# juwangvsu/cartographer-1

Measured on AMD Instinct MI355X. Metric: loop-closure constraint candidates/sec (node x submap pairs) + ms/scan-match, 2D 5cm grid, higher is better.
Workload: dtype u8

## Files before the change

cartographer-1_amd/csrc/csm_device.h:

```cpp
#ifndef CSM_DEVICE_H_
#define CSM_DEVICE_H_

#include <cstdint>

#if defined(__HIPCC__)
#define CSM_HD __host__ __device__
#else
#define CSM_HD
#endif

namespace csm {

constexpr int kMaxLevels = 12;
constexpr int kNumXcd = 8;
constexpr int kSearchThreads = 256;
constexpr int kWaves = kSearchThreads / 64;
constexpr int kStackCap = 160;
constexpr int kTopChunk = 64;
constexpr int kMaxPoints = 16448;
constexpr int kIndexLimit = 16383;
constexpr int kOffsetLimit = 8191;
constexpr int kMaxRotations = 16383;
constexpr int16_t kSentinel = -32768;

struct SubmapDesc {
  double max_x, max_y, resolution;
  int32_t nx, ny;
  int32_t levels;
  int32_t pad0;
  const uint8_t* level[kMaxLevels];
  int32_t wide_nx[kMaxLevels];
  int32_t wide_ny[kMaxLevels];
  int32_t zero_index[kMaxLevels];
  const uint32_t* quad[kMaxLevels];
  const uint8_t* pyramid_base;
  int32_t pyramid_bytes;
  int32_t quad_off[kMaxLevels];
  int32_t quad_pws[kMaxLevels];
  int32_t quad_pph[kMaxLevels];
  int32_t quad_w[kMaxLevels];
  int32_t quad_h[kMaxLevels];
  int32_t quad_bytes[kMaxLevels];
  int32_t cshift[kMaxLevels];
  int32_t quad_bias[kMaxLevels];
  int32_t quad_es[kMaxLevels];
  int32_t hex_mask;
};

constexpr int kMaxClusterShift = 3;

constexpr int kHexEntryBytes = 16;

struct PairDesc {
  int32_t submap;
  int32_t num_points;
  int64_t point_offset;
  int32_t rot_offset;
  int32_t num_scans;
  int32_t num_linear;
  int32_t max_rejected_sum;
  float tx, ty;
  float pre_w, pre_s;
  int32_t collect;
  int32_t collect_sum;
};

struct ScoreJob {
  int32_t pair, rot, first, count;
};
constexpr int kTieCap = 4096;

struct WalkJob2 {
  int32_t pair;
  int32_t target_sum;
  int32_t top_level;
  int32_t top_first;
  int32_t top_count;
  int32_t bounds_first;
  float min_s, max_s;
};
constexpr int kWalkStack = 64;

struct WorkQueues {
  const int32_t* pair_order;
  const int64_t* chunk_prefix;
  int32_t queue_begin[kNumXcd + 1];
  int64_t queue_chunks[kNumXcd];
  int32_t rot_chunk;
};

struct WorkQueues2 {
  const int32_t* pair_order;
  const int64_t* chunk_prefix;
  const int32_t* block_first;
  int32_t block_offset[kNumXcd];
  int32_t queue_begin[kNumXcd + 1];
  int64_t queue_chunks[kNumXcd];
  int32_t rot_chunk;
};

#ifndef CSM_MAX_ROT_CHUNK
#define CSM_MAX_ROT_CHUNK 16
#endif
constexpr int kV4MaxRotChunk = CSM_MAX_ROT_CHUNK;

constexpr int kStack2 = 1024;
constexpr int kSpill2 = 7168;
constexpr int kBatchNodes = 64;

constexpr int kSumShift = 42;
constexpr uint64_t kTieMask = (uint64_t(1) << kSumShift) - 1;

CSM_HD inline uint64_t PackLeafKey(uint32_t sum, int rot, int xo, int yo) {
  const uint64_t idx = (uint64_t(rot) << 28) | (uint64_t(xo + 8192) << 14) |
                       uint64_t(yo + 8192);
  return (uint64_t(sum) << kSumShift) | (~idx & kTieMask);
}
CSM_HD inline uint64_t HighLeafKey(uint64_t key) {
  return (key & ~kTieMask) | (~key & kTieMask);
}
CSM_HD inline void UnpackLeafKey(uint64_t key, uint32_t* sum, int* rot, int* xo, int* yo) {
  *sum = static_cast<uint32_t>(key >> kSumShift);
  const uint64_t idx = ~key & kTieMask;
  *rot = static_cast<int>(idx >> 28);
  *xo = static_cast<int>((idx >> 14) & 0x3fff) - 8192;
  *yo = static_cast<int>(idx & 0x3fff) - 8192;
}

constexpr int kStatHighWater = 2 + 2 * kMaxLevels + 4;
constexpr int kStatLines = kStatHighWater + 1;
constexpr int kStatsWords = kStatLines + 5 * kMaxLevels;

constexpr int32_t kStatusRange = 1;

}

#endif
```

cartographer-1_amd/csrc/csm_host.cc:

```cpp

#include <hip/hip_runtime.h>

#include <algorithm>
#include <atomic>
#include <chrono>
#include <cmath>
#include <cstdlib>
#include <cstring>
#include <limits>
#include <map>
#include <memory>
#include <mutex>
#include <set>
#include <thread>
#include <array>
#include <tuple>
#include <vector>

#include "../../include/csm_amd.h"
#include "csm_device.h"
#include "csm_internal.h"
#include "csm_launch.h"
#include "parallel_sort.h"
#include "search_window.h"

namespace csm {



namespace {


int AutoSearchDepth(int configured, int nx, int ny) {
  int d = configured;
  const int span = std::max(nx, ny);
  while (d < kMaxLevels && (1 << (d - 1)) < span / 2) ++d;
  return std::max(d, configured);
}

void ClusterShifts(int32_t* out) {
  static const int kDefault[kMaxLevels] = {0, 0, 2, 2, 2, 3, 3, 3, 3, 3, 3, 3};
  for (int l = 0; l < kMaxLevels; ++l) out[l] = kDefault[l];
  if (const char* env = std::getenv("CSM_CLUSTER")) {
    int l = 0;
    for (const char* c = env; *c && l < kMaxLevels; ++l) {
      out[l] = std::atoi(c);
      while (*c && *c != ',') ++c;
      if (*c == ',') ++c;
    }
    for (; l < kMaxLevels; ++l) out[l] = out[l - 1];
  }
  for (int l = 0; l < kMaxLevels; ++l)
    out[l] = std::max(0, std::min({out[l], l, kMaxClusterShift}));
}

}
}

using namespace csm;


namespace {

int EnsureDevice(csm_context* ctx) {
  return hipSetDevice(ctx->device) == hipSuccess ? CSM_OK : CSM_EHIP;
}

}

namespace csm {

namespace {
std::mutex& PoolRegistryMutex() {
  static std::mutex m;
  return m;
}
std::vector<BufPool*>& PoolRegistry() {
  static std::vector<BufPool*> r;
  return r;
}
}

BufPool::BufPool() {
  std::lock_guard<std::mutex> g(PoolRegistryMutex());
  PoolRegistry().push_back(this);
}

BufPool::~BufPool() {
  {
    std::lock_guard<std::mutex> g(PoolRegistryMutex());
    auto& r = PoolRegistry();
    r.erase(std::remove(r.begin(), r.end(), this), r.end());
  }
  Release();
}

void BufPool::Release() {
  std::lock_guard<std::mutex> g(mu_);
  for (auto& b : bufs_) (void)hipFree(b.first);
  bufs_.clear();
  held_ = 0;
}

int BufPool::Take(size_t n, DevBuf* out) {
  {
    std::lock_guard<std::mutex> g(mu_);
    int best = -1;
    for (int i = 0; i < static_cast<int>(bufs_.size()); ++i) {
      const size_t b = bufs_[i].second;
      if (b >= n && b <= 2 * n + 4096 && (best < 0 || b < bufs_[best].second)) best = i;
    }
    if (best >= 0) {
      out->ptr = bufs_[best].first;
      out->bytes = bufs_[best].second;
      held_ -= bufs_[best].second;
      bufs_.erase(bufs_.begin() + best);
      return CSM_OK;
    }
  }
  return out->Reserve(n);
}

void BufPool::Give(DevBuf* b) {
  constexpr size_t kMaxPooled = 8192;
  if (!b->ptr) return;
  std::lock_guard<std::mutex> g(mu_);
  bufs_.emplace_back(b->ptr, b->bytes);
  held_ += b->bytes;
  b->ptr = nullptr;
  b->bytes = 0;
  size_t drop = 0;
  while (drop < bufs_.size() && (bufs_.size() - drop > kMaxPooled || held_ > cap_bytes_)) {
    held_ -= bufs_[drop].second;
    (void)hipFree(bufs_[drop].first);
    ++drop;
  }
  bufs_.erase(bufs_.begin(), bufs_.begin() + static_cast<std::ptrdiff_t>(drop));
}

void ReleaseIdlePools() {
  std::lock_guard<std::mutex> g(PoolRegistryMutex());
  for (BufPool* p : PoolRegistry()) p->Release();
}

csm_context* AcquireCallContext(csm_context* owner) {
  {
    std::lock_guard<std::mutex> g(owner->call_mu);
    if (!owner->call_free.empty()) {
      csm_context* c = owner->call_free.back();
      owner->call_free.pop_back();
      c->timing = owner->timing.load();
      return c;
    }
  }
  csm_context* c = nullptr;
  if (csm_context_create(owner->device, &c) != CSM_OK) return nullptr;
  c->call_owner = owner;
  c->timing = owner->timing.load();
  std::lock_guard<std::mutex> g(owner->call_mu);
  owner->call_all.push_back(c);
  return c;
}

void ReleaseCallContext(csm_context* owner, csm_context* c) {
  if (!c) return;
  std::lock_guard<std::mutex> g(owner->call_mu);
  AddTiming(&owner->call_t, c->t);
  c->t = csm_timing{};
  owner->call_free.push_back(c);
}

}

namespace {

const std::pair<SearchWindow2D, std::vector<ZRot>>& WindowFor(
    csm_scan_set* s, int scan, double lin, double ang, double res) {
  const auto key = std::make_tuple(scan, ang, lin, res);
  auto it = s->windows.find(key);
  if (it != s->windows.end()) return it->second;
  const int64_t b = s->offsets[scan], e = s->offsets[scan + 1];
  SearchWindow2D w = MakeSearchWindow2D(lin, ang, s->host_points.data() + 3 * b,
                                        static_cast<int32_t>(e - b), res, nullptr);
  std::vector<ZRot> table;
  RotationTable(w, &table);
  return s->windows.emplace(key, std::make_pair(w, std::move(table))).first->second;
}

struct SearchPlan {
  bool use_v2 = true, hex = false, fifo = true;
  int rc = 2, max_npad = 64;
};

int LaunchSearch(csm_context* ctx, csm_scan_set* scans, const std::vector<PairDesc>& pdesc,
                 const std::vector<uint64_t>* init_best, const SearchPlan& plan, bool timed,
                 std::vector<uint64_t>* keys, std::vector<uint64_t>* keys_hi,
                 std::vector<int32_t>* stat, unsigned long long* stats_host,
                 std::vector<uint2>* ties = nullptr, std::vector<int32_t>* tie_counts = nullptr) {
  const int np = static_cast<int>(pdesc.size());
  const int rc = plan.rc;
  static const bool spread_on = [] {
    const char* e = std::getenv("CSM_QUEUE_SPREAD");
    return !(e && std::atoi(e) == 0);
  }();
  int nsub = 0;
  for (int i = 0; i < np; ++i) nsub = std::max(nsub, pdesc[i].submap + 1);
  const int reps = spread_on && nsub > 0 && nsub < kNumXcd ? kNumXcd / nsub : 1;
  std::vector<int32_t> seen(reps > 1 ? nsub : 0, 0);
  std::vector<std::vector<int32_t>> q(kNumXcd);
  for (int i = 0; i < np; ++i) {
    const int sm = pdesc[i].submap;
    const int qi = reps > 1 ? sm + nsub * (seen[sm]++ % reps) : sm % kNumXcd;
    q[qi].push_back(i);
  }
  std::vector<int32_t> order;
  std::vector<int64_t> prefix;
  WorkQueues wq{};
  wq.rot_chunk = rc;
  int64_t running = 0;
  for (int x = 0; x < kNumXcd; ++x) {
    std::stable_sort(q[x].begin(), q[x].end(),
                     [&](int a, int b) { return pdesc[a].submap < pdesc[b].submap; });
    wq.queue_begin[x] = static_cast<int32_t>(order.size());
    const int64_t qstart = running;
    for (int pi : q[x]) {
      order.push_back(pi);
      prefix.push_back(running);
      running += (pdesc[pi].num_scans + rc - 1) / rc;
    }
    wq.queue_chunks[x] = running - qstart;
  }
  wq.queue_begin[kNumXcd] = static_cast<int32_t>(order.size());
  prefix.push_back(running);

  std::vector<int32_t> blocks;
  WorkQueues2 wq2{};
  if (plan.use_v2) {
    wq2.rot_chunk = rc;
    for (int x = 0; x < kNumXcd; ++x) {
      wq2.queue_begin[x] = wq.queue_begin[x];
      wq2.queue_chunks[x] = wq.queue_chunks[x];
      wq2.block_offset[x] = static_cast<int32_t>(blocks.size());
      const int64_t qstart = prefix[wq.queue_begin[x]];
      int e = wq.queue_begin[x];
      for (int64_t c = 0; c < wq.queue_chunks[x]; c += 64) {
        while (prefix[e + 1] - qstart <= c) ++e;
        blocks.push_back(e);
      }
    }
    wq2.queue_begin[kNumXcd] = wq.queue_begin[kNumXcd];
  }

  auto align = [](size_t v) { return (v + 255) & ~size_t{255}; };
  size_t at = 0;
  auto region = [&](size_t bytes) {
    const size_t o = at;
    at = align(at + std::max<size_t>(bytes, 1));
    return o;
  };
  const size_t o_pd = region(sizeof(PairDesc) * np), o_order = region(sizeof(int32_t) * order.size()),
               o_prefix = region(sizeof(int64_t) * prefix.size()),
               o_blocks = region(sizeof(int32_t) * blocks.size());
  const size_t o_best = region(sizeof(uint64_t) * np), o_hi = region(sizeof(uint64_t) * np),
               o_status = region(sizeof(int32_t) * np), o_tcount = region(sizeof(int32_t) * np),
               o_counters = region(sizeof(unsigned long long) * kNumXcd);
  const size_t o_stats = region(sizeof(unsigned long long) * kStatsWords);
  const size_t arena_bytes = at;
  const size_t in_end = init_best ? o_hi : o_best;
  const size_t zero_begin = in_end;
  int rcode;
  if ((rcode = ctx->arena.Reserve(arena_bytes))) return rcode;
  if ((rcode = ctx->arena_in.Reserve(in_end))) return rcode;
  if ((rcode = ctx->arena_out.Reserve(arena_bytes - o_best))) return rcode;
  if (ties && (rcode = ctx->ties.Reserve(sizeof(uint2) * kTieCap * static_cast<size_t>(np))))
    return rcode;
  char* hin = ctx->arena_in.as<char>();
  std::memcpy(hin + o_pd, pdesc.data(), sizeof(PairDesc) * np);
  std::memcpy(hin + o_order, order.data(), sizeof(int32_t) * order.size());
  std::memcpy(hin + o_prefix, prefix.data(), sizeof(int64_t) * prefix.size());
  if (!blocks.empty()) std::memcpy(hin + o_blocks, blocks.data(), sizeof(int32_t) * blocks.size());
  if (init_best) std::memcpy(hin + o_best, init_best->data(), sizeof(uint64_t) * np);
  char* dev = ctx->arena.as<char>();
  hipStream_t st = ctx->stream;
  CSM_HIP(hipMemcpyAsync(dev, hin, in_end, hipMemcpyHostToDevice, st));
  CSM_HIP(hipMemsetAsync(dev + zero_begin, 0, arena_bytes - zero_begin, st));
  ctx->pair_desc_dev = dev + o_pd;
  PairDesc* d_pairs = reinterpret_cast<PairDesc*>(dev + o_pd);
  uint64_t* d_best = reinterpret_cast<uint64_t*>(dev + o_best);
  uint64_t* d_hi = reinterpret_cast<uint64_t*>(dev + o_hi);
  int32_t* d_status = reinterpret_cast<int32_t*>(dev + o_status);
  int32_t* d_tcount = reinterpret_cast<int32_t*>(dev + o_tcount);
  unsigned long long* d_counters = reinterpret_cast<unsigned long long*>(dev + o_counters);
  unsigned long long* d_stats = reinterpret_cast<unsigned long long*>(dev + o_stats);
  wq.pair_order = reinterpret_cast<int32_t*>(dev + o_order);
  wq.chunk_prefix = reinterpret_cast<int64_t*>(dev + o_prefix);

  const int64_t total_chunks = running;
  const int max_npad = plan.max_npad;
  if (timed) CSM_HIP(hipEventRecord(ctx->ev0, st));
  if (plan.use_v2) {
    wq2.pair_order = wq.pair_order;
    wq2.chunk_prefix = wq.chunk_prefix;
    wq2.block_first = reinterpret_cast<int32_t*>(dev + o_blocks);
    int capc = (3 * max_npad / 4 + 63) & ~63;
    if (const char* ce = std::getenv("CSM_CAPC_PCT"))
      capc = std::max(64, (std::atoi(ce) * max_npad / 100 + 63) & ~63);
    const int lds_cap = 96 * 1024;
    auto dyn_bytes = [&](int cap) { return static_cast<size_t>(rc) * (max_npad * 4 + cap * 5); };
    while (capc > 0 && dyn_bytes(capc) > lds_cap) capc -= 64;
    const size_t dyn_lds = (dyn_bytes(capc) + 15) & ~size_t{15};
    int per_cu = std::max(1, std::min(8, Fast2dSearchV2BlocksPerCu(plan.hex, plan.fifo, dyn_lds)));
    if (const char* w = std::getenv("CSM_WG_PER_CU")) per_cu = std::max(1, std::min(per_cu, std::atoi(w)));
    if (std::getenv("CSM_PROFILE2D") && !init_best)
      std::fprintf(stderr, "fast2d launch: %s %s, %d rotations per item, %zu B dynamic LDS (capc %d), %d workgroups per CU\n",
                   plan.hex ? "v5" : "v4", plan.fifo ? "fifo" : "lifo", rc, dyn_lds, capc, per_cu);
    const int64_t full = static_cast<int64_t>(ctx->num_cus) * per_cu;
    const int64_t share = std::max<int64_t>(ctx->num_cus, full / std::max(1, ctx->grid_share));
    const int grid = static_cast<int>(std::min<int64_t>(share, std::max<int64_t>(total_chunks, 1)));
    if ((rcode = ctx->spill.Reserve(sizeof(uint2) * kSpill2 * static_cast<size_t>(grid))))
      return rcode;
    CSM_HIP(LaunchFast2dSearchV2(grid, dyn_lds, st, ctx->submap_desc.as<SubmapDesc>(), d_pairs,
                                 scans->points.as<float>(), scans->rot_dev.as<float2>(), wq2,
                                 d_counters, d_best, d_status, d_stats, ctx->spill.as<uint2>(),
                                 max_npad, capc, plan.hex, plan.fifo, d_hi,
                                 ties ? ctx->ties.as<uint2>() : nullptr, d_tcount, ties != nullptr));
  } else {
    const size_t dyn_lds = static_cast<size_t>(rc) * max_npad * sizeof(uint32_t);
    const int grid = static_cast<int>(std::min<int64_t>(static_cast<int64_t>(ctx->num_cus) * 4,
                                                        std::max<int64_t>(total_chunks, 1)));
    CSM_HIP(LaunchFast2dSearch(grid, dyn_lds, st, ctx->submap_desc.as<SubmapDesc>(), d_pairs,
                               scans->points.as<float>(), scans->rot_dev.as<float2>(), wq,
                               d_counters, d_best, d_status, d_stats));
  }
  if (timed) CSM_HIP(hipEventRecord(ctx->ev1, st));
  char* hout = ctx->arena_out.as<char>();
  CSM_HIP(hipMemcpyAsync(hout, dev + o_best, arena_bytes - o_best, hipMemcpyDeviceToHost, st));
  if (ties) {
    ties->resize(static_cast<size_t>(kTieCap) * np);
    CSM_HIP(hipMemcpyAsync(ties->data(), ctx->ties.ptr, sizeof(uint2) * ties->size(),
                           hipMemcpyDeviceToHost, st));
  }
  CSM_HIP(hipStreamSynchronize(st));
  auto out = [&](size_t o) { return hout + (o - o_best); };
  keys->assign(reinterpret_cast<uint64_t*>(out(o_best)), reinterpret_cast<uint64_t*>(out(o_best)) + np);
  keys_hi->assign(reinterpret_cast<uint64_t*>(out(o_hi)), reinterpret_cast<uint64_t*>(out(o_hi)) + np);
  stat->assign(reinterpret_cast<int32_t*>(out(o_status)), reinterpret_cast<int32_t*>(out(o_status)) + np);
  std::memcpy(stats_host, out(o_stats), sizeof(unsigned long long) * kStatsWords);
  if (ties)
    tie_counts->assign(reinterpret_cast<int32_t*>(out(o_tcount)),
                       reinterpret_cast<int32_t*>(out(o_tcount)) + np);
  return CSM_OK;
}

void RotationBounds(const csm_scan_set* scans, const PairDesc& d, const SubmapDesc& sm,
                    const ZRot& rot, int b[4]) {
  int mnx = 0x7fffffff, mxx = -0x7fffffff, mny = 0x7fffffff, mxy = -0x7fffffff;
  const ZRot pre{d.pre_w, d.pre_s};
  const float* p = scans->host_points.data() + 3 * d.point_offset;
  for (int i = 0; i < d.num_points; ++i) {
    float x, y;
    RotateZ(pre, p[3 * i], p[3 * i + 1], &x, &y);
    RotateZ(rot, x, y, &x, &y);
    const float px = d.tx + x, py = d.ty + y;
    const int ix = static_cast<int>(std::round((sm.max_y - static_cast<double>(py)) / sm.resolution - 0.5));
    const int iy = static_cast<int>(std::round((sm.max_x - static_cast<double>(px)) / sm.resolution - 0.5));
    mnx = std::min(mnx, ix); mxx = std::max(mxx, ix);
    mny = std::min(mny, iy); mxy = std::max(mxy, iy);
  }
  b[0] = std::max(-d.num_linear, std::min(0, -mxx));
  b[1] = std::min(d.num_linear, std::max(0, sm.nx - 1 - mnx));
  b[2] = std::max(-d.num_linear, std::min(0, -mxy));
  b[3] = std::min(d.num_linear, std::max(0, sm.ny - 1 - mny));
}

int ResolveTies(csm_context* ctx, csm_fast2d* const* submaps, csm_scan_set* scans,
                const std::vector<PairDesc>& pdesc, const std::vector<float2>& rot_host,
                const SearchPlan& plan, std::vector<int32_t>* stat,
                const std::vector<uint64_t>& keys_hi, std::vector<uint64_t>* keys,
                std::vector<int8_t>* tie_code) {
  std::vector<int> tied;
  for (int k = 0; k < static_cast<int>(pdesc.size()); ++k) {
    const uint64_t key = (*keys)[k];
    if (((*stat)[k] & kStatusRange) || key == 0) continue;
    const int64_t sum = static_cast<int64_t>(key >> kSumShift);
    if (sum <= pdesc[k].max_rejected_sum) continue;
    if ((keys_hi[k] >> kSumShift) == (key >> kSumShift) && keys_hi[k] != HighLeafKey(key))
      tied.push_back(k);
  }
  if (tied.empty()) return CSM_OK;
  ctx->t.tied_pairs += static_cast<int64_t>(tied.size());
  const bool prof = std::getenv("CSM_PROFILE2D") != nullptr;
  auto now = [] { return std::chrono::steady_clock::now(); };
  auto ms = [](std::chrono::steady_clock::time_point a, std::chrono::steady_clock::time_point b) {
    return std::chrono::duration<double, std::milli>(b - a).count();
  };
  const auto tp0 = now();
  std::vector<PairDesc> pd2;
  std::vector<uint64_t> init;
  for (int k : tied) {
    PairDesc d = pdesc[k];
    d.collect = 1;
    d.collect_sum = static_cast<int32_t>((*keys)[k] >> kSumShift);
    pd2.push_back(d);
    init.push_back(static_cast<uint64_t>(d.collect_sum) << kSumShift);
  }
  std::vector<uint64_t> k2, kh2;
  std::vector<int32_t> st2, counts;
  std::vector<uint2> ties;
  unsigned long long stats2[kStatsWords] = {0};
  int rc;
  if ((rc = LaunchSearch(ctx, scans, pd2, &init, plan, false, &k2, &kh2, &st2, stats2, &ties,
                         &counts)))
    return rc;
  auto zrot = [&](const PairDesc& d, int r) {
    const float2 z = rot_host[d.rot_offset + r];
    return ZRot{z.x, z.y};
  };
  struct Tie {
    int k, t, depth, leaves_first, leaves_count;
  };
  std::vector<Tie> work;
  std::vector<int3> leaves;
  std::vector<ScoreJob> jobs;
  std::vector<int4> queries;
  std::vector<int> leaf_query;
  std::vector<int> walk;
  for (size_t t = 0; t < tied.size(); ++t) {
    const int k = tied[t];
    const int cnt = counts[t];
    if ((st2[t] & kStatusRange) || cnt > kTieCap || cnt < 2) {
      ctx->t.ties_walked += 1;
      (*tie_code)[k] = CSM_TIE_WALK;
      walk.push_back(static_cast<int>(t));
      continue;
    }
    const PairDesc& d = pdesc[k];
    const csm_fast2d* m = submaps[d.submap];
    Tie w{k, static_cast<int>(t), m->options.branch_and_bound_depth,
          static_cast<int>(leaves.size()), cnt};
    std::map<int, std::vector<int>> by_rot;
    for (int i = 0; i < cnt; ++i) {
      const uint2 e = ties[static_cast<size_t>(t) * kTieCap + i];
      const int r = static_cast<int>(e.x);
      const int x = static_cast<int16_t>(e.y & 0xffff), y = static_cast<int>(e.y) >> 16;
      leaves.push_back(make_int3(r, x, y));
      by_rot[r].push_back(w.leaves_first + i);
    }
    leaf_query.resize(leaves.size(), -1);
    const int T = w.depth - 1;
    for (auto& [r, idx] : by_rot) {
      int b[4];
      RotationBounds(scans, d, m->desc, zrot(d, r), b);
      if (T < 1) continue;
      ScoreJob job{static_cast<int32_t>(t), r, static_cast<int32_t>(queries.size()), 0};
      for (int li : idx) {
        leaf_query[li] = static_cast<int>(queries.size());
        for (int lv = 1; lv <= T; ++lv) {
          const int ax = b[0] + (((leaves[li].y - b[0]) >> lv) << lv);
          const int ay = b[2] + (((leaves[li].z - b[2]) >> lv) << lv);
          queries.push_back(make_int4(lv, ax, ay, 0));
        }
      }
      job.count = static_cast<int32_t>(queries.size()) - job.first;
      jobs.push_back(job);
    }
    work.push_back(w);
  }
  auto score = [&](const std::vector<ScoreJob>& js, const std::vector<int4>& qs,
// ... 1158 lines not shown
```

cartographer-1_amd/csrc/csm_kernels.hip:

```cpp

#include <hip/hip_runtime.h>

#include <algorithm>

#include "csm_device.h"
#include "geom2d_dev.h"

namespace csm {


__device__ __forceinline__ int WaveSum(int v) {
#pragma unroll
  for (int m = 32; m >= 1; m >>= 1) v += __shfl_xor(v, m, 64);
  return v;
}
__device__ __forceinline__ int WaveMin(int v) {
#pragma unroll
  for (int m = 32; m >= 1; m >>= 1) v = min(v, __shfl_xor(v, m, 64));
  return v;
}
__device__ __forceinline__ int WaveMax(int v) {
#pragma unroll
  for (int m = 32; m >= 1; m >>= 1) v = max(v, __shfl_xor(v, m, 64));
  return v;
// ... 750 lines not shown
  #pragma unroll
      for (int u = 0; u < U; ++u) {
        const int idx = i + u * groups + g;
        const bool in = idx < len;
        const int j = in ? idx : 0;
        ad[u] = address(P[j], in);
        c[u] = in ? (raw ? 1u : Cn[j]) : 0u;
      }
      for (int u = 0; u < U; ++u) CSM_COUNT_LINES(level, ad[u], kOOB);
      HexVec v[U];
  #pragma unroll
      for (int u = 0; u < U; ++u) v[u] = hload(ad[u]);
  #pragma unroll
      for (int u = 0; u < U; ++u) accumulate(v[u], c[u]);
    }
    for (; i < e; i += groups) {
      const int idx = i + g;
      const bool in = idx < e && idx < len;
      const int j = in ? idx : 0;
      const HexVec vv = hload(address(P[j], in));
      accumulate(vv, in ? (raw ? 1u : Cn[j]) : 0u);
    }
  }
  if (active) {
#pragma unroll
    for (int j = 0; j < 16; ++j)
      if (acc[j] != 0u) atomicAdd(&sh.part[Shared::PartIndex(node, j)], static_cast<int>(acc[j]));
  }
}

__device__ __forceinline__ uint32_t ClusterKey(uint32_t p, int shift) {
  const int x = (static_cast<int16_t>(p & 0xffff) >> shift) << shift;
  const int y = ((static_cast<int>(p) >> 16) >> shift) << shift;
  return (static_cast<uint32_t>(x) & 0xffff) | (static_cast<uint32_t>(y) << 16);
}

template <bool kWrite>
__device__ int RunList(const uint32_t* src, int n, uint32_t mask, uint32_t* P, uint8_t* C) {
  const int lane = threadIdx.x & 63;
  const unsigned long long upto = (2ull << lane) - 1;
  int out = 0, run_start = 0, open_k = -1, open_pos = 0;
  uint32_t last = 0;
  uint32_t nextv = lane < n ? src[lane] : 0u;
  for (int base = 0; base < n; base += 64) {
    const int i = base + lane;
    const bool in = i < n;
    const uint32_t v = nextv;
    nextv = i + 64 < n ? src[i + 64] : 0u;
    uint32_t prev = static_cast<uint32_t>(__builtin_amdgcn_update_dpp(
        0, static_cast<int>(v), 0x138, 0xF, 0xF, false));
    if (lane == 0) prev = last;
    const bool head0 = in && (i == 0 || ((v ^ prev) & mask) != 0u);
    const unsigned long long h0 = __ballot(head0);
    unsigned long long hm = h0;
    if (base + 63 - run_start >= 255) {
      const unsigned long long mine = h0 & upto;
      const int rs = mine ? base + 63 - __clzll(mine) : run_start;
      hm = __ballot(head0 || (in && i > rs && (i - rs) % 255 == 0));
    }
    if (kWrite) {
      if (open_k >= 0 && hm) {
        if (lane == 0) C[open_k] = static_cast<uint8_t>(base + __ffsll(static_cast<long long>(hm)) - 1 - open_pos);
        open_k = -1;
      }
      if ((hm >> lane) & 1ull) {
        const int k = out + static_cast<int>(__builtin_amdgcn_mbcnt_hi(
                                static_cast<uint32_t>(hm >> 32),
                                __builtin_amdgcn_mbcnt_lo(static_cast<uint32_t>(hm), 0u)));
        P[k] = v & mask;
        const unsigned long long rest = lane < 63 ? hm >> (lane + 1) : 0ull;
        if (rest) C[k] = static_cast<uint8_t>(__ffsll(static_cast<long long>(rest)));
      }
      if (hm) {
        open_k = out + __popcll(hm) - 1;
        open_pos = base + 63 - __clzll(hm);
      }
    }
    out += __popcll(hm);
    if (h0) run_start = base + 63 - __clzll(h0);
    last = __builtin_amdgcn_readlane(v, 63);
  }
  if (kWrite && open_k >= 0 && lane == 0) C[open_k] = static_cast<uint8_t>(n - open_pos);
  return out;
}

__device__ __forceinline__ uint32_t ClusterMask(int sl) {
  const uint32_t h = (0xffffu << sl) & 0xffffu;
  return h | (h << 16);
}

#ifndef CSM_BEST_REFRESH
#define CSM_BEST_REFRESH 1
#endif
#ifndef CSM_LIFO_LEVEL
#define CSM_LIFO_LEVEL 2
#endif
#ifndef CSM_XFAST
#define CSM_XFAST 1
#endif
#ifndef CSM_ORIGIN_ALIGN
#define CSM_ORIGIN_ALIGN 8
#endif
static_assert((CSM_ORIGIN_ALIGN & (CSM_ORIGIN_ALIGN - 1)) == 0, "CSM_ORIGIN_ALIGN: a power of two");
#ifndef CSM_TIE_PRUNE
#define CSM_TIE_PRUNE 1
#endif
#ifndef CSM_V4_WAVES
#define CSM_V4_WAVES 6
#endif
template <bool kHex, bool kFifo, bool kCollect>
__global__ void __launch_bounds__(kSearchThreads) __attribute__((amdgpu_waves_per_eu(CSM_V4_WAVES)))
fast2d_search_v4(const SubmapDesc* __restrict__ submaps,
                 const PairDesc* __restrict__ pairs,
                 const float* __restrict__ points,
                 const float2* __restrict__ rot_table,
                 WorkQueues2 queues,
                 unsigned long long* __restrict__ counters,
                 uint64_t* __restrict__ best,
                 int32_t* __restrict__ status,
                 unsigned long long* __restrict__ stats,
                 uint2* __restrict__ spill_base, int npad, int capc,
                 uint64_t* __restrict__ best_hi, uint2* __restrict__ ties,
                 int32_t* __restrict__ tie_count) {
  constexpr int kKids = kHex ? 16 : 4;
  extern __shared__ __align__(16) uint32_t cells[];
  __shared__ V4Shared<kKids> sh;
  const int tid = threadIdx.x, lane = tid & 63, wave = tid >> 6;
  const int rc = queues.rot_chunk;
  uint8_t* cnts = reinterpret_cast<uint8_t*>(cells + rc * (npad + capc));
  const int raw_end = rc * npad;
  uint2* spill = spill_base + static_cast<size_t>(blockIdx.x) * kSpill2;
  for (int k = tid; k < kBatchNodes * kKids; k += kSearchThreads) sh.part[k] = 0;
  if (tid == 0) sh.batch_hex = 0;
  if (tid == 0) sh.high_water = 0;
  unsigned long long local_cands = 0, local_lookups = 0;
#ifdef CSM_KPROF
  long long kprof[4] = {0, 0, 0, 0};
#endif
  if (tid == 0) sh.queue = blockIdx.x % kNumXcd;
  unsigned long long lv_cands = 0, lv_batches = 0;
#ifdef CSM_KPROF
  if (tid < kMaxLevels) {
    sh.kp_lines[tid] = 0; sh.kp_instr[tid] = 0; sh.kp_qlines[tid] = 0;
    sh.kp_active[tid] = 0; sh.kp_oob[tid] = 0;
  }
#endif
  int tries = 0;
  __syncthreads();
  for (;;) {
    if (tid == 0) {
      int q = sh.queue, pair = -1, chunk = 0;
      while (tries < kNumXcd) {
        const int64_t item = static_cast<int64_t>(atomicAdd(&counters[q], 1ull));
        if (item < queues.queue_chunks[q]) {
          const int64_t gch = queues.chunk_prefix[queues.queue_begin[q]] + item;
          int e = queues.block_first[queues.block_offset[q] + static_cast<int>(item >> 6)];
          while (queues.chunk_prefix[e + 1] <= gch) ++e;
          pair = queues.pair_order[e];
          chunk = static_cast<int>(gch - queues.chunk_prefix[e]);
          break;
        }
        q = (q + 1) % kNumXcd;
        ++tries;
      }
      sh.queue = q;
      sh.item_pair = pair;
      sh.item_chunk = chunk;
    }
    __syncthreads();
    const int pair_index = Uniform(sh.item_pair);
    if (pair_index < 0) break;
    const PairDesc pd = pairs[pair_index];
    const SubmapDesc& sm = submaps[pd.submap];
    const int n = pd.num_points;
    const int s_min = pd.max_rejected_sum;
    const int collect_sum = kCollect ? pd.collect_sum : -1;
    uint64_t* pair_best = best + pair_index;
    const int rot0 = Uniform(sh.item_chunk) * rc;
    const int nrot = min(rc, pd.num_scans - rot0);
    const int top_level = sm.levels - 1;
    const int step = 1 << top_level;
    const uint32_t hex_mask = kHex ? static_cast<uint32_t>(Uniform(sm.hex_mask)) : 0u;

#ifdef CSM_KPROF
    long long t_mark = clock64();
#endif
    if (tid < kMaxRotChunk * 4) sh.mm[tid >> 2][tid & 3] = (tid & 1) ? -0x7fffffff : 0x7fffffff;
    if (tid == 0) sh.range_error = 0;
    if (tid < sm.levels) {
      const int d = tid;
      sh.lv[d][0] = sm.quad_w[d];
      sh.lv[d][1] = sm.quad_h[d];
      sh.lv[d][2] = sm.quad_off[d];
      sh.lv[d][3] = sm.quad_pws[d] * sm.quad_es[d];
      sh.lv[d][4] = sm.quad_pws[d] * sm.quad_pph[d] * sm.quad_es[d];
      sh.lv[d][5] = sm.quad_bias[d];
      sh.lv[d][6] = sm.cshift[d];
    }
    __syncthreads();
    const double inv_res = 1.0 / sm.resolution;
    bool range_error = false;
    for (int r = 0; r < nrot; ++r) {
      const float2 q = rot_table[pd.rot_offset + rot0 + r];
      int mnx = 0x7fffffff, mxx = -0x7fffffff, mny = 0x7fffffff, mxy = -0x7fffffff;
      for (int i = tid; i < n; i += kSearchThreads) {
        const float* p = points + 3 * (pd.point_offset + i);
        float x, y;
        RotateZDev(pd.pre_w, pd.pre_s, p[0], p[1], &x, &y);
        RotateZDev(q.x, q.y, x, y, &x, &y);
        const float px = __fadd_rn(pd.tx, x);
        const float py = __fadd_rn(pd.ty, y);
        const double cx = CellCoordFast(sm.max_y, py, sm.resolution, inv_res);
        const double cy = CellCoordFast(sm.max_x, px, sm.resolution, inv_res);
        int ix = 0, iy = 0;
        if (fabs(cx) > kIndexLimit || fabs(cy) > kIndexLimit) {
          range_error = true;
        } else {
          ix = static_cast<int>(cx);
          iy = static_cast<int>(cy);
        }
        mnx = min(mnx, ix); mxx = max(mxx, ix);
        mny = min(mny, iy); mxy = max(mxy, iy);
        cells[r * npad + i] = (static_cast<uint32_t>(ix) & 0xffff) | (static_cast<uint32_t>(iy) << 16);
      }
      mnx = WaveMin(mnx); mxx = WaveMax(mxx); mny = WaveMin(mny); mxy = WaveMax(mxy);
      if (lane == 0) {
        atomicMin(&sh.mm[r][0], mnx); atomicMax(&sh.mm[r][1], mxx);
        atomicMin(&sh.mm[r][2], mny); atomicMax(&sh.mm[r][3], mxy);
      }
    }
    if (range_error) sh.range_error = 1;
#ifdef CSM_DBG
    if (range_error) printf("discretize range\n");
#endif
    __syncthreads();
    {
#ifdef CSM_KPROF
      const long long t_lists = clock64();
#endif
      if (tid < nrot * kLists) sh.list_len[tid / kLists][tid % kLists] = tid % kLists == 0 ? n : 0;
      if (tid == 0) sh.long_runs = 0;
      __syncthreads();
      for (int r = 0; r < nrot; ++r) {
        const uint32_t* raw = cells + r * npad;
        uint32_t c1 = 0, c23 = 0;
        bool long_run = false;
        for (int i = tid; i < n; i += kSearchThreads) {
          const uint32_t v = raw[i];
          const uint32_t d = i == 0 ? 0xffffffffu : v ^ raw[i - 1];
          c1 += (d & ClusterMask(1)) != 0u;
          c23 += ((d & ClusterMask(2)) != 0u) | (static_cast<uint32_t>((d & ClusterMask(3)) != 0u) << 16);
          long_run |= i >= 255 && ((v ^ raw[i - 255]) & ClusterMask(kMaxClusterShift)) == 0u;
        }
        c1 = DppSum(c1);
        c23 = DppSum(c23);
        if (lane == 0) {
          atomicAdd(&sh.list_len[r][1], static_cast<int>(c1));
          atomicAdd(&sh.list_len[r][2], static_cast<int>(c23 & 0xffff));
          atomicAdd(&sh.list_len[r][3], static_cast<int>(c23 >> 16));
        }
        if (__ballot(long_run) && lane == 0) atomicOr(&sh.long_runs, 1 << r);
      }
      __syncthreads();
      if (const int lr = sh.long_runs) {
        for (int t = wave; t < nrot * kMaxClusterShift; t += kWaves) {
          const int r = t / kMaxClusterShift, sl = 1 + t % kMaxClusterShift;
          if (lr >> r & 1) {
            const int len = RunList<false>(cells + r * npad, n, ClusterMask(sl), nullptr, nullptr);
            if (lane == 0) sh.list_len[r][sl] = len;
          }
        }
        __syncthreads();
      }
      uint32_t used_sl = 0;
      for (int d = 0; d < sm.levels; ++d) used_sl |= 1u << sh.lv[d][6];
      if (tid < nrot) {
        const int r = tid;
        sh.list_off[r][0] = r * npad;
        int used = 0;
        int off[kLists] = {r * npad, -1, -1, -1};
        for (int sl = kMaxClusterShift; sl >= 1; --sl)
          if ((used_sl >> sl & 1u) && used + sh.list_len[r][sl] <= capc) {
            off[sl] = rc * npad + r * capc + used;
            used += sh.list_len[r][sl];
          }
        for (int sl = 1; sl < kLists; ++sl) {
          if (off[sl] >= 0) {
            sh.list_off[r][sl] = off[sl];
          } else {
            sh.list_off[r][sl] = sh.list_off[r][sl - 1];
            sh.list_len[r][sl] = sh.list_len[r][sl - 1] | (1 << 30);
          }
        }
      }
      __syncthreads();
      const int nused = __popc(used_sl & 0xeu);
      for (int t = wave; t < nrot * nused; t += kWaves) {
        const int r = t / nused;
        int sl = 0;
        for (int k = t % nused, m = used_sl & 0xe; k >= 0; --k) {
          sl = __ffs(m) - 1;
          m &= m - 1;
        }
        if (!(sh.list_len[r][sl] & (1 << 30)))
          RunList<true>(cells + r * npad, n, ClusterMask(sl), cells + sh.list_off[r][sl],
                        cnts + (sh.list_off[r][sl] - raw_end));
      }
      __syncthreads();
      if (tid < nrot * kLists) sh.list_len[tid / kLists][tid % kLists] &= ~(1 << 30);
      __syncthreads();
#ifdef CSM_KPROF
      if (tid == 0) kprof[3] += clock64() - t_lists;
// ... 629 lines not shown
```

Measured before the change: 14380.

## Interleave pair chunks via rectangle schedule with golden-ratio strides

Replaces the per-queue sequential pair/chunk list with a schedule that groups same-submap pairs into blocks, sorts them by chunk count, and packs them into rectangles. Consecutive work items then round-robin across pairs instead of draining one pair at a time, and chunk order inside a pair is permuted with a golden-ratio stride. The aim is to spread concurrent workgroups across many pairs and rotation ranges, so shared best-score pruning tightens sooner and per-pair contention drops. The cost is a few empty slots that need extra atomic retries, a more expensive device-side slot decode with a division, and host time to build the schedule.

```diff
diff --git a/cartographer-1_amd/csrc/csm_device.h b/cartographer-1_amd/csrc/csm_device.h
--- a/cartographer-1_amd/csrc/csm_device.h
+++ b/cartographer-1_amd/csrc/csm_device.h
@@ -89,15 +89,43 @@
   int32_t rot_chunk;
 };
 
+struct SchedEntry {
+  int32_t pair;
+  int32_t chunks;
+  int32_t stride;
+  int32_t pad;
+};
+struct SchedRect {
+  int64_t slot_begin, slot_end;
+  int32_t first;
+  int32_t width;
+  int32_t pos0;
+  int32_t pad;
+};
 struct WorkQueues2 {
-  const int32_t* pair_order;
-  const int64_t* chunk_prefix;
-  const int32_t* block_first;
-  int32_t block_offset[kNumXcd];
-  int32_t queue_begin[kNumXcd + 1];
-  int64_t queue_chunks[kNumXcd];
+  const SchedEntry* entries;
+  const SchedRect* rects;
+  const int32_t* hint;
+  int32_t hint_offset[kNumXcd];
+  int64_t queue_slots[kNumXcd];
+  int32_t hint_shift;
   int32_t rot_chunk;
 };
+
+CSM_HD inline bool DecodeSlot(const WorkQueues2& w, int q, int64_t slot, int* pair, int* chunk) {
+  int r = w.hint[w.hint_offset[q] + static_cast<int>(slot >> w.hint_shift)];
+  SchedRect rect = w.rects[r];
+  while (slot >= rect.slot_end) rect = w.rects[++r];
+  const uint32_t rel = static_cast<uint32_t>(slot - rect.slot_begin);
+  const uint32_t width = static_cast<uint32_t>(rect.width);
+  const uint32_t row = rel / width;
+  const SchedEntry e = w.entries[rect.first + static_cast<int>(rel - row * width)];
+  const uint32_t pos = static_cast<uint32_t>(rect.pos0) + row;
+  if (pos >= static_cast<uint32_t>(e.chunks)) return false;
+  *pair = e.pair;
+  *chunk = static_cast<int>(pos * static_cast<uint32_t>(e.stride) % static_cast<uint32_t>(e.chunks));
+  return true;
+}
 
 #ifndef CSM_MAX_ROT_CHUNK
 #define CSM_MAX_ROT_CHUNK 16
diff --git a/cartographer-1_amd/csrc/csm_host.cc b/cartographer-1_amd/csrc/csm_host.cc
--- a/cartographer-1_amd/csrc/csm_host.cc
+++ b/cartographer-1_amd/csrc/csm_host.cc
@@ -21,6 +21,7 @@
 #include "csm_device.h"
 #include "csm_internal.h"
 #include "csm_launch.h"
+#include "csm_schedule.h"
 #include "parallel_sort.h"
 #include "search_window.h"
 
@@ -203,52 +204,39 @@
     const char* e = std::getenv("CSM_QUEUE_SPREAD");
     return !(e && std::atoi(e) == 0);
   }();
-  int nsub = 0;
-  for (int i = 0; i < np; ++i) nsub = std::max(nsub, pdesc[i].submap + 1);
-  const int reps = spread_on && nsub > 0 && nsub < kNumXcd ? kNumXcd / nsub : 1;
-  std::vector<int32_t> seen(reps > 1 ? nsub : 0, 0);
-  std::vector<std::vector<int32_t>> q(kNumXcd);
+  std::vector<int32_t> pair_submap(np), pair_chunks(np);
   for (int i = 0; i < np; ++i) {
-    const int sm = pdesc[i].submap;
-    const int qi = reps > 1 ? sm + nsub * (seen[sm]++ % reps) : sm % kNumXcd;
-    q[qi].push_back(i);
-  }
+    pair_submap[i] = pdesc[i].submap;
+    pair_chunks[i] = (pdesc[i].num_scans + rc - 1) / rc;
+  }
+  const std::vector<std::vector<int32_t>> q = AssignQueues(pair_submap, spread_on);
   std::vector<int32_t> order;
   std::vector<int64_t> prefix;
   WorkQueues wq{};
   wq.rot_chunk = rc;
-  int64_t running = 0;
-  for (int x = 0; x < kNumXcd; ++x) {
-    std::stable_sort(q[x].begin(), q[x].end(),
-                     [&](int a, int b) { return pdesc[a].submap < pdesc[b].submap; });
-    wq.queue_begin[x] = static_cast<int32_t>(order.size());
-    const int64_t qstart = running;
-    for (int pi : q[x]) {
-      order.push_back(pi);
-      prefix.push_back(running);
-      running += (pdesc[pi].num_scans + rc - 1) / rc;
-    }
-    wq.queue_chunks[x] = running - qstart;
-  }
-  wq.queue_begin[kNumXcd] = static_cast<int32_t>(order.size());
-  prefix.push_back(running);
-
-  std::vector<int32_t> blocks;
-  WorkQueues2 wq2{};
+  Schedule sched;
+  int64_t total_chunks = 0;
+  double sched_ms = 0.0;
   if (plan.use_v2) {
-    wq2.rot_chunk = rc;
+    const auto t0 = std::chrono::steady_clock::now();
+    sched = BuildSchedule(q, pair_submap, pair_chunks, rc);
+    sched_ms = std::chrono::duration<double, std::milli>(std::chrono::steady_clock::now() - t0).count();
+    total_chunks = sched.items;
+  } else {
+    int64_t running = 0;
     for (int x = 0; x < kNumXcd; ++x) {
-      wq2.queue_begin[x] = wq.queue_begin[x];
-      wq2.queue_chunks[x] = wq.queue_chunks[x];
-      wq2.block_offset[x] = static_cast<int32_t>(blocks.size());
-      const int64_t qstart = prefix[wq.queue_begin[x]];
-      int e = wq.queue_begin[x];
-      for (int64_t c = 0; c < wq.queue_chunks[x]; c += 64) {
-        while (prefix[e + 1] - qstart <= c) ++e;
-        blocks.push_back(e);
+      wq.queue_begin[x] = static_cast<int32_t>(order.size());
+      const int64_t qstart = running;
+      for (int pi : q[x]) {
+        order.push_back(pi);
+        prefix.push_back(running);
+        running += (pdesc[pi].num_scans + rc - 1) / rc;
       }
-    }
-    wq2.queue_begin[kNumXcd] = wq.queue_begin[kNumXcd];
+      wq.queue_chunks[x] = running - qstart;
+    }
+    wq.queue_begin[kNumXcd] = static_cast<int32_t>(order.size());
+    prefix.push_back(running);
+    total_chunks = running;
   }
 
   auto align = [](size_t v) { return (v + 255) & ~size_t{255}; };
@@ -258,9 +246,12 @@
     at = align(at + std::max<size_t>(bytes, 1));
     return o;
   };
-  const size_t o_pd = region(sizeof(PairDesc) * np), o_order = region(sizeof(int32_t) * order.size()),
-               o_prefix = region(sizeof(int64_t) * prefix.size()),
-               o_blocks = region(sizeof(int32_t) * blocks.size());
+  const size_t o_pd = region(sizeof(PairDesc) * np);
+  const size_t o_order = region(plan.use_v2 ? sizeof(SchedEntry) * sched.entries.size()
+                                            : sizeof(int32_t) * order.size()),
+               o_prefix = region(plan.use_v2 ? sizeof(SchedRect) * sched.rects.size()
+                                             : sizeof(int64_t) * prefix.size()),
+               o_blocks = region(sizeof(int32_t) * sched.hint.size());
   const size_t o_best = region(sizeof(uint64_t) * np), o_hi = region(sizeof(uint64_t) * np),
                o_status = region(sizeof(int32_t) * np), o_tcount = region(sizeof(int32_t) * np),
                o_counters = region(sizeof(unsigned long long) * kNumXcd);
@@ -276,9 +267,14 @@
     return rcode;
   char* hin = ctx->arena_in.as<char>();
   std::memcpy(hin + o_pd, pdesc.data(), sizeof(PairDesc) * np);
-  std::memcpy(hin + o_order, order.data(), sizeof(int32_t) * order.size());
-  std::memcpy(hin + o_prefix, prefix.data(), sizeof(int64_t) * prefix.size());
-  if (!blocks.empty()) std::memcpy(hin + o_blocks, blocks.data(), sizeof(int32_t) * blocks.size());
+  if (plan.use_v2) {
+    std::memcpy(hin + o_order, sched.entries.data(), sizeof(SchedEntry) * sched.entries.size());
+    std::memcpy(hin + o_prefix, sched.rects.data(), sizeof(SchedRect) * sched.rects.size());
+    std::memcpy(hin + o_blocks, sched.hint.data(), sizeof(int32_t) * sched.hint.size());
+  } else {
+    std::memcpy(hin + o_order, order.data(), sizeof(int32_t) * order.size());
+    std::memcpy(hin + o_prefix, prefix.data(), sizeof(int64_t) * prefix.size());
+  }
   if (init_best) std::memcpy(hin + o_best, init_best->data(), sizeof(uint64_t) * np);
   char* dev = ctx->arena.as<char>();
   hipStream_t st = ctx->stream;
@@ -295,13 +291,13 @@
   wq.pair_order = reinterpret_cast<int32_t*>(dev + o_order);
   wq.chunk_prefix = reinterpret_cast<int64_t*>(dev + o_prefix);
 
-  const int64_t total_chunks = running;
   const int max_npad = plan.max_npad;
   if (timed) CSM_HIP(hipEventRecord(ctx->ev0, st));
   if (plan.use_v2) {
-    wq2.pair_order = wq.pair_order;
-    wq2.chunk_prefix = wq.chunk_prefix;
-    wq2.block_first = reinterpret_cast<int32_t*>(dev + o_blocks);
+    WorkQueues2 wq2 = sched.wq;
+    wq2.entries = reinterpret_cast<SchedEntry*>(dev + o_order);
+    wq2.rects = reinterpret_cast<SchedRect*>(dev + o_prefix);
+    wq2.hint = reinterpret_cast<int32_t*>(dev + o_blocks);
     int capc = (3 * max_npad / 4 + 63) & ~63;
     if (const char* ce = std::getenv("CSM_CAPC_PCT"))
       capc = std::max(64, (std::atoi(ce) * max_npad / 100 + 63) & ~63);
@@ -312,8 +308,12 @@
     int per_cu = std::max(1, std::min(8, Fast2dSearchV2BlocksPerCu(plan.hex, plan.fifo, dyn_lds)));
     if (const char* w = std::getenv("CSM_WG_PER_CU")) per_cu = std::max(1, std::min(per_cu, std::atoi(w)));
     if (std::getenv("CSM_PROFILE2D") && !init_best)
-      std::fprintf(stderr, "fast2d launch: %s %s, %d rotations per item, %zu B dynamic LDS (capc %d), %d workgroups per CU\n",
-                   plan.hex ? "v5" : "v4", plan.fifo ? "fifo" : "lifo", rc, dyn_lds, capc, per_cu);
+      std::fprintf(stderr, "fast2d launch: %s %s, %d rotations per item, %zu B dynamic LDS (capc %d), %d workgroups per CU; "
+                   "%lld items, %lld empty slots (%.3f %%), %zu rectangles, %zu hints, built in %.3f ms\n",
+                   plan.hex ? "v5" : "v4", plan.fifo ? "fifo" : "lifo", rc, dyn_lds, capc, per_cu,
+                   static_cast<long long>(sched.items), static_cast<long long>(sched.empty_slots),
+                   100.0 * sched.empty_slots / std::max<int64_t>(sched.items, 1), sched.rects.size(),
+                   sched.hint.size(), sched_ms);
     const int64_t full = static_cast<int64_t>(ctx->num_cus) * per_cu;
     const int64_t share = std::max<int64_t>(ctx->num_cus, full / std::max(1, ctx->grid_share));
     const int grid = static_cast<int>(std::min<int64_t>(share, std::max<int64_t>(total_chunks, 1)));
diff --git a/cartographer-1_amd/csrc/csm_kernels.hip b/cartographer-1_amd/csrc/csm_kernels.hip
--- a/cartographer-1_amd/csrc/csm_kernels.hip
+++ b/cartographer-1_amd/csrc/csm_kernels.hip
@@ -926,12 +926,8 @@
       int q = sh.queue, pair = -1, chunk = 0;
       while (tries < kNumXcd) {
         const int64_t item = static_cast<int64_t>(atomicAdd(&counters[q], 1ull));
-        if (item < queues.queue_chunks[q]) {
-          const int64_t gch = queues.chunk_prefix[queues.queue_begin[q]] + item;
-          int e = queues.block_first[queues.block_offset[q] + static_cast<int>(item >> 6)];
-          while (queues.chunk_prefix[e + 1] <= gch) ++e;
-          pair = queues.pair_order[e];
-          chunk = static_cast<int>(gch - queues.chunk_prefix[e]);
+        if (item < queues.queue_slots[q]) {
+          if (!DecodeSlot(queues, q, item, &pair, &chunk)) continue;
           break;
         }
         q = (q + 1) % kNumXcd;
diff --git a/cartographer-1_amd/csrc/csm_schedule.h b/cartographer-1_amd/csrc/csm_schedule.h
--- /dev/null
+++ b/cartographer-1_amd/csrc/csm_schedule.h
@@ -0,0 +1,166 @@
+#ifndef CSM_SCHEDULE_H_
+#define CSM_SCHEDULE_H_
+
+#include <algorithm>
+#include <cstdint>
+#include <initializer_list>
+#include <numeric>
+#include <vector>
+
+#include "csm_device.h"
+
+#ifndef CSM_SCHED_BLOCK
+#define CSM_SCHED_BLOCK 256
+#endif
+#ifndef CSM_SCHED_GOLDEN
+#define CSM_SCHED_GOLDEN 1
+#endif
+
+namespace csm {
+
+inline std::vector<std::vector<int32_t>> AssignQueues(const std::vector<int32_t>& submap,
+                                                      bool spread) {
+  const int np = static_cast<int>(submap.size());
+  int nsub = 0;
+  for (int i = 0; i < np; ++i) nsub = std::max(nsub, submap[i] + 1);
+  const int reps = spread && nsub > 0 && nsub < kNumXcd ? kNumXcd / nsub : 1;
+  std::vector<int32_t> seen(reps > 1 ? nsub : 0, 0);
+  std::vector<std::vector<int32_t>> q(kNumXcd);
+  for (int i = 0; i < np; ++i) {
+    const int sm = submap[i];
+    const int qi = reps > 1 ? sm + nsub * (seen[sm]++ % reps) : sm % kNumXcd;
+    q[qi].push_back(i);
+  }
+  for (auto& v : q)
+    std::stable_sort(v.begin(), v.end(), [&](int a, int b) { return submap[a] < submap[b]; });
+  return q;
+}
+
+inline int32_t GoldenStrideSearch(int32_t chunks) {
+  if (chunks <= 2) return 1;
+  const int32_t s0 = static_cast<int32_t>(chunks * 0.6180339887498949 + 0.5);
+  int32_t best = 1, best_q = chunks + 1;
+  for (int32_t d = 0; d <= 8; ++d)
+    for (int32_t s : {s0 + d, s0 - d}) {
+      if (s < 1 || s >= chunks) continue;
+      int32_t a = chunks, b = s, q = 0;
+      while (b > 0) {
+        q = std::max(q, a / b);
+        const int32_t r = a % b;
+        a = b;
+        b = r;
+      }
+      if (a == 1 && q < best_q) best = s, best_q = q;
+    }
+  return best;
+}
+inline int32_t GoldenStride(int32_t chunks) {
+  static const std::vector<int32_t> table = [] {
+    std::vector<int32_t> t(kMaxRotations + 1);
+    for (int32_t n = 0; n <= kMaxRotations; ++n) t[n] = GoldenStrideSearch(n);
+    return t;
+  }();
+  return chunks >= 0 && chunks <= kMaxRotations ? table[chunks] : GoldenStrideSearch(chunks);
+}
+
+struct Schedule {
+  std::vector<SchedEntry> entries;
+  std::vector<SchedRect> rects;
+  std::vector<int32_t> hint;
+  WorkQueues2 wq{};
+  int64_t items = 0;
+  int64_t empty_slots = 0;
+};
+
+inline int64_t CutBlock(const int32_t* c, int n, int64_t cap, int32_t first, int64_t* slot,
+                        std::vector<SchedRect>* out) {
+  int64_t empty = 0;
+  int32_t pos = 0;
+  for (;;) {
+    while (n > 0 && c[n - 1] <= pos) --n;
+    if (n == 0) break;
+    int m = n - 1;
+    int64_t waste = 0;
+    while (m > 0) {
+      const int64_t more = waste + static_cast<int64_t>(n - m) * (c[m - 1] - c[m]);
+      if (more > cap) break;
+      waste = more;
+      --m;
+    }
+    const int32_t top = c[m];
+    if (out) {
+      SchedRect r{};
+      r.slot_begin = *slot;
+      r.slot_end = *slot + static_cast<int64_t>(n) * (top - pos);
+      r.first = first;
+      r.width = n;
+      r.pos0 = pos;
+      out->push_back(r);
+      *slot = r.slot_end;
+    }
+    empty += waste;
+    pos = top;
+  }
+  return empty;
+}
+
+inline Schedule BuildSchedule(const std::vector<std::vector<int32_t>>& queues,
+                              const std::vector<int32_t>& submap,
+                              const std::vector<int32_t>& chunks, int rot_chunk,
+                              int block_pairs = CSM_SCHED_BLOCK, bool golden = CSM_SCHED_GOLDEN) {
+  Schedule s;
+  s.wq.rot_chunk = rot_chunk;
+  block_pairs = std::max(1, std::min(block_pairs, 1 << 16));
+  std::vector<int32_t> run, counts;
+  std::vector<int32_t> queue_rect_begin(kNumXcd + 1, 0);
+  int64_t max_slots = 0;
+  for (int x = 0; x < kNumXcd; ++x) {
+    queue_rect_begin[x] = static_cast<int32_t>(s.rects.size());
+    const std::vector<int32_t>& q = queues[x];
+    int64_t slot = 0;
+    for (size_t b = 0; b < q.size();) {
+      size_t e = b;
+      while (e < q.size() && submap[q[e]] == submap[q[b]]) ++e;
+      run.assign(q.begin() + b, q.begin() + e);
+      std::stable_sort(run.begin(), run.end(),
+                       [&](int a, int c) { return chunks[a] > chunks[c]; });
+      for (size_t k = 0; k < run.size(); k += block_pairs) {
+        const int n = static_cast<int>(std::min<size_t>(block_pairs, run.size() - k));
+        const int32_t first = static_cast<int32_t>(s.entries.size());
+        counts.clear();
+        int64_t items = 0;
+        for (int i = 0; i < n; ++i) {
+          const int32_t pair = run[k + i], c = chunks[pair];
+          s.entries.push_back(SchedEntry{pair, c, golden ? GoldenStride(c) : 1, 0});
+          counts.push_back(c);
+          items += c;
+        }
+        const int64_t budget = items / 100;
+        int64_t cap = budget;
+        while (CutBlock(counts.data(), n, cap, first, nullptr, nullptr) > budget) cap /= 2;
+        s.empty_slots += CutBlock(counts.data(), n, cap, first, &slot, &s.rects);
+        s.items += items;
+      }
+      b = e;
+    }
+    s.wq.queue_slots[x] = slot;
+    max_slots = std::max(max_slots, slot);
+  }
+  queue_rect_begin[kNumXcd] = static_cast<int32_t>(s.rects.size());
+  int shift = 6;
+  while ((max_slots >> shift) >= 1024) ++shift;
+  s.wq.hint_shift = shift;
+  for (int x = 0; x < kNumXcd; ++x) {
+    s.wq.hint_offset[x] = static_cast<int32_t>(s.hint.size());
+    int r = queue_rect_begin[x];
+    for (int64_t at = 0; at < s.wq.queue_slots[x]; at += int64_t{1} << shift) {
+      while (s.rects[r].slot_end <= at) ++r;
+      s.hint.push_back(r);
+    }
+  }
+  return s;
+}
+
+}
+
+#endif
```

New measurement: 14880 (median of 6 runs). +3.4%, better.
